# Juleszwanen/oscar_mpc_planner_mr_modification

Hardware: AMD Instinct MI355X
Metric: SQP solves/s (N=20, 8 obs, 8 guesses) at 1/2/4/8 MI355X; max |x−x_ref| (higher is better)
Workload: dtype f64

## Files before the change

### oscar_mpc_planner_mr_modification_amd/csrc/mpcg_sqp.h

```cpp
#pragma once
#include <hip/hip_runtime.h>

#include <type_traits>

#include "mpcg.h"
#include "mpcg_bicycle.h"
#include "mpcg_device.h"

namespace mpcg {

enum { AC_SUCCESS = 0, AC_NAN = 1, AC_MAXITER = 2, AC_MINSTEP = 3, AC_QP_FAILURE = 4 };

__host__ __device__ constexpr int imax(int a, int b) { return a > b ? a : b; }
__host__ __device__ constexpr int sym(int i, int j) { return i >= j ? i * (i + 1) / 2 + j : j * (j + 1) / 2 + i; }
__host__ __device__ constexpr int cpk(int n, int a, int c) { return c * n - c * (c - 1) / 2 + (a - c); }

__host__ __device__ constexpr int lds_b64_cycles(int s, int off, int parts) {
    int total = 0;
    for (int half = 0; half < 2; ++half) {
        int dw[64] = {};
        int n = 0;
        for (int l = 32 * half; l < 32 * half + 32; ++l) {
            const int a = 2 * (s * (l / parts) + off * (l % parts));
            for (int h = 0; h < 2; ++h) {
// ... 40 lines not shown
#endif
    static constexpr int NPTP = (MPCG_P_PAD && MODEL_ != 1 && (64 / (N_ + 1)) >= 3) ? NPT + (NPT & 1) : NPT;
    static constexpr int NB = (HAS_SLACK && NS > 0) ? 4 : 3;
    static constexpr int NBT = NB * (NB + 1) / 2;
    static constexpr int NDH = NZ + NBT + 1;
#ifndef MPCG_PARTS_BIKE
#define MPCG_PARTS_BIKE 2
#endif
    static constexpr int PARTS_MAX = (64 / (N + 1)) >= 3 ? 3 : 2;
    static constexpr int PARTS = MODEL_ == 1 ? (MPCG_PARTS_BIKE < PARTS_MAX ? MPCG_PARTS_BIKE : PARTS_MAX) : PARTS_MAX;
    static_assert((N + 1) * PARTS <= 64, "horizon too long for one wavefront");
    static_assert(NTRI <= 64, "stage block larger than a wavefront");
#if defined(MPCG_NO_QUEUE)
    static constexpr bool QUEUE = false;
#elif defined(MPCG_QUEUE_ALL)
    static constexpr bool QUEUE = true;
#else
    static constexpr bool QUEUE = MODEL_ == 0 && PARTS_MAX == 3;
#endif
    static constexpr int BVS = (NZ + PARTS - 1) / PARTS;
    static constexpr int HS = (NH + PARTS - 1) / PARTS;
    static constexpr int SLOTS = 2 * BVS + HS;
#ifndef MPCG_STORE_IT_MAX
#define MPCG_STORE_IT_MAX 13
#endif
#ifndef MPCG_STORE_IT_MAX2
#ifdef MPCG_STORE_IT_ANY
#define MPCG_STORE_IT_MAX2 12
#else
#define MPCG_STORE_IT_MAX2 0
#endif
#endif
    static constexpr bool STORE_IT = SLOTS <= (PARTS == 3 ? MPCG_STORE_IT_MAX : MPCG_STORE_IT_MAX2);
#ifndef MPCG_BOUNDS_SEL
#define MPCG_BOUNDS_SEL 0
#endif
    static constexpr bool BOUNDS_SEL = MPCG_BOUNDS_SEL > 0;
    static constexpr int NBOX = 2 * NU + 2 * NX;
#ifdef MPCG_LIN_PARAMS_ALL
    static constexpr bool LIN_PARAMS = true;
#else
    static constexpr bool LIN_PARAMS = NS > 0 || N >= 30;
#endif
    static constexpr int DGC = LIN_PARAMS ? 2 : 3;
    static constexpr int NHS = LIN_PARAMS ? (NE > 0 ? NE : 1) : NH;
    static constexpr bool RELOAD_PARAMS = NS > 0 || N >= 30;
    static constexpr int M_TOTAL = 2 * NU + (N - 1) * (NBOX + NH);
    __host__ __device__ static constexpr int blk(int v) {
        return (v >= IX && v <= IPSI) ? v - IX : ((NB == 4 && v == ZSL) ? 3 : -1);
    }
    __host__ __device__ static constexpr int bvar(int b) { return b < 3 ? IX + b : ZSL; }
    static constexpr bool COMPACT = MODEL_ == 1;
#ifndef MPCG_FCONST_N
#define MPCG_FCONST_N 30
#endif
    static constexpr bool FCONST = MODEL_ == 0 && N_ >= MPCG_FCONST_N;
    static constexpr int NFR = COMPACT ? 4 : (FCONST ? 2 : NX), NFC = COMPACT ? NZ - 1 : NZ;
    static constexpr int NHP = COMPACT ? (NZ - 1) * NZ / 2 + 1 : NTRI;
#ifndef MPCG_C3_SPLIT
#define MPCG_C3_SPLIT 0
#endif
#ifndef MPCG_C3_FACFLAT
#define MPCG_C3_FACFLAT 0
#endif
    static constexpr bool CHAIN_SPLIT = !COMPACT || MPCG_C3_SPLIT;
#if defined(MPCG_NO_PAIR)
    static constexpr bool PAIR_WANTED = false;
#elif defined(MPCG_PAIR_ALL)
    static constexpr bool PAIR_WANTED = true;
#else
    static constexpr bool PAIR_WANTED = FCONST && NE_ <= 8;
#endif
    static constexpr bool PAIR_CHAINS = PAIR_WANTED && CHAIN_SPLIT && (N_ + 1) / 2 * NX_ * NX_ <= (N_ + 1) * NDH &&
                                        (N_ + 1) / 2 * NX_ <= 128;
    static constexpr bool FAC_FLAT = !COMPACT || MPCG_C3_FACFLAT;
#ifndef MPCG_REC_P2
#define MPCG_REC_P2 0
#endif
#ifdef MPCG_REC_SELECT
    static constexpr bool REC_FLAT = CHAIN_SPLIT && PARTS == 3;
#else
    static constexpr bool REC_FLAT = CHAIN_SPLIT && (PARTS == 3 || MPCG_REC_P2);
#endif
    static constexpr int QPM_ROWS = 2 * SLOTS * 64;
    static constexpr int QPM = QPM_ROWS + (N + 1) * NZ + N * NX;
    __host__ __device__ static constexpr double slack_coef(int hh) { return (NB == 4 && hh >= NL + NE) ? -1.0 : 0.0; }
};

template <class C, bool LEAN = C::COMPACT, bool GFH = false, int PAD = 0>
struct Lds {
    static constexpr int N = C::N, NX = C::NX, NZ = C::NZ;
    static constexpr int DGS =
        PAD ? lds_stride(C::NHS * C::DGC, C::DGC, C::PARTS, C::DGC % 2 == 0 ? 2 : 1, 3) : C::NHS * C::DGC;
    static constexpr int HDS = PAD ? lds_stride(C::NHS, 1, C::PARTS, 1, 3) : C::NHS;
    static constexpr int PS = PAD == 0   ? C::NPTP
                              : PAD == 2 ? lds_stride(C::NPT + (C::NPT & 1), 0, C::PARTS, 2, 4)
                                         : lds_stride(C::NPTP, 0, C::PARTS, C::NPTP == C::NPT ? 1 : 2, 4);
    double z[N + 1][NZ];
    double H[GFH ? 1 : N + 1][C::NHP];
    double g[N + 1][NZ];
    double F[GFH ? 1 : N][C::NFR][C::NFC];
    double Fst[GFH && !C::COMPACT ? C::NFR : 1][C::NFC];
    double Hst[GFH && !C::COMPACT ? C::NHP : 1];
    double b[N][NX];
    double dH[N + 1][C::NDH];
    double q[N + 1][NZ];
    double dz[N + 1][NZ];
    double ddz[N + 1][NZ];
    double pi_nlp[N][NX];
    double piq[N][NX];
    double pin[LEAN ? 1 : N][NX];
    double rdyn[LEAN ? 1 : N][NX];
    alignas(16) double P[N + 1][PS];
    double Lc[N][C::NLC];
    double Y[N][C::NU][NX];
    double bx[N + 1][NZ];
    double Dg[N][DGS];
    double hd[N][HDS];
    double disc[C::LIN_PARAMS ? N : 1][4];
    double Msc[128];
    double xinit[NX];
    int flag;
};

#ifdef MPCG_LDS_SOLVES_PER_CU
constexpr size_t LDS_QUARTER = 160 * 1024 / MPCG_LDS_SOLVES_PER_CU;
constexpr bool LDS_SMALLEST = true;
#else
constexpr size_t LDS_QUARTER = 160 * 1024 / 4;
constexpr bool LDS_SMALLEST = false;
#endif
template <class C>
__host__ __device__ constexpr bool lds_lean() {
    if (LDS_SMALLEST) return C::COMPACT || sizeof(Lds<C, false>) > LDS_QUARTER;
    return C::COMPACT || (sizeof(Lds<C, false>) > LDS_QUARTER && sizeof(Lds<C, true>) <= LDS_QUARTER);
}
template <class C>
__host__ __device__ constexpr bool lds_gfh() {
#ifdef MPCG_NO_GFH
    return false;
#else
    if (LDS_SMALLEST) return sizeof(Lds<C, lds_lean<C>(), false>) > LDS_QUARTER;
    return sizeof(Lds<C, lds_lean<C>(), false>) > LDS_QUARTER && sizeof(Lds<C, lds_lean<C>(), true>) <= LDS_QUARTER;
#endif
}
template <class C>
__host__ __device__ constexpr int lds_pad() {
#if defined(MPCG_NO_STRIDE_PAD)
    return 0;
#else
#if defined(MPCG_NO_P_ALIGN)
    constexpr bool P_ALIGN = false;
#else
    constexpr bool P_ALIGN = !C::COMPACT;
#endif
    return P_ALIGN && sizeof(Lds<C, lds_lean<C>(), lds_gfh<C>(), 2>) <= LDS_QUARTER ? 2
           : sizeof(Lds<C, lds_lean<C>(), lds_gfh<C>(), 1>) <= LDS_QUARTER         ? 1
                                                                                   : 0;
#endif
}
template <class C>
using LdsOf = Lds<C, lds_lean<C>(), lds_gfh<C>(), lds_pad<C>()>;
template <class C>
__host__ __device__ constexpr size_t gfh_doubles() {
    return lds_gfh<C>() ? (size_t)C::N * C::NFR * C::NFC + (size_t)(C::N + 1) * C::NHP : 0;
}
// ... 333 lines not shown
```

### oscar_mpc_planner_mr_modification_amd/csrc/mpcg_sqp_body.inc

```
    constexpr int N = C::N, PARTS = C::PARTS, NX = C::NX, NZ = C::NZ, NB = C::NB, NBT = C::NBT;
    constexpr int NU = C::NU;
    constexpr int ZS = C::ZSL;
    constexpr int X0 = C::IX, X1 = C::IY, X2 = C::IPSI;
    constexpr bool LEAN = lds_lean<C>();
    constexpr bool GFH = lds_gfh<C>();
#ifndef MPCG_FUSE_BAR
#define MPCG_FUSE_BAR 1
#endif
    constexpr bool FUSE_BAR = MPCG_FUSE_BAR > 0;
#ifndef MPCG_COND
#define MPCG_COND 1
#endif
#ifndef MPCG_ITREF
#define MPCG_ITREF 1
#endif
#ifndef MPCG_MOVE
#define MPCG_MOVE 1
#endif
#ifndef MPCG_RES_SPLIT
#define MPCG_RES_SPLIT 1
#endif
    constexpr bool RES_SPLIT = MPCG_RES_SPLIT > 0 && FUSE_BAR && !C::COMPACT && PARTS > 1 && 2 * NB <= NZ &&
                               ((PARTS == 3 && NX == 5) || MPCG_RES_SPLIT > 1);
    constexpr int DRS = (NX + PARTS - 1) / PARTS;
    static_assert(!(RES_SPLIT && LEAN), "the split passes read the dynamics multipliers from S.pin");
#if defined(MPCG_CENTRED_FLAG)
    constexpr bool CFLAG = MPCG_CENTRED_FLAG > 0;
#else
    constexpr bool CFLAG = !LEAN && !C::HAS_SLACK;
#endif
#ifndef MPCG_MSPLIT
#define MPCG_MSPLIT 0
#endif
    constexpr bool MSPLIT = MPCG_MSPLIT > 0 && C::MODEL == 0;
#ifndef MPCG_PIN_SPLIT
#define MPCG_PIN_SPLIT 0
#endif
    constexpr bool PIN_SPLIT = MPCG_PIN_SPLIT > 0 && RES_SPLIT && !LEAN && C::CHAIN_SPLIT;
    __shared__ LdsOf<C> S;
#ifdef MPCG_LDS_PAD
    __shared__ char lds_pad[MPCG_LDS_PAD];
    if (threadIdx.x == 1000) lds_pad[blockIdx.x % MPCG_LDS_PAD] = 0;
#endif
    if (sol >= batch) return;
    if (blockDim.x != 64) {
        if (threadIdx.x == 0) io.exit_code[sol] = -1;
        return;
    }
#ifdef MPCG_LDS_POISON
    for (int e = threadIdx.x; e < (int)(sizeof(S) / 8); e += 64) ((double*)&S)[e] = __builtin_nan("");
    wave_sync();
#endif
    int lane_ = threadIdx.x;
    if constexpr (C::QUEUE) __asm__ volatile("" : "+v"(lane_));
    const int lane = lane_;
    const int k = lane / PARTS;
    const int part = lane - k * PARTS;
    const bool stage_lane = (part == 0) && (k <= N);
    const int ks = k <= N ? k : N;
    const int kc = k < N ? k : N - 1;
    const int npar = pr.npar;
    constexpr int LAMS = NX + C::NH;
#ifdef MPCG_DIAG_PARAMS_OF
    const double* pbase = io.params + (size_t)(sol % MPCG_DIAG_PARAMS_OF) * N * npar;
#else
    const double* pbase = io.params + (size_t)sol * N * npar;
#endif
    const double* pk = pbase + (size_t)kc * npar;
    (void)stamps;
    constexpr bool SPLIT = MODE != MODE_FUSED;
    double* const gsol = gws + (size_t)(SPLIT ? sol : (int)blockIdx.x) * ws_doubles<C>();
    double* const gF = GFH ? gsol : nullptr;
    double* const g_ddz0 = gsol + gfh_doubles<C>();
    double* const g_pin0 = g_ddz0 + (N + 1) * NZ;
    double* const g_dz0 = g_pin0 + N * NX;
    double* const gH = GFH ? gF + (size_t)N * C::NFR * C::NFC : nullptr;
    auto Fb = [&](int kq) -> double (*)[C::NFC] {
        if constexpr (GFH) return (double (*)[C::NFC])(gF + (size_t)kq * C::NFR * C::NFC);
        else return S.F[kq];
    };
    auto Hb = [&](int kq) -> double* {
        if constexpr (GFH) return gH + (size_t)kq * C::NHP;
        else return S.H[kq];
    };
    STAMP_DECL
    using CB = Carry<C>;
    double* const gcar = g_ddz0 + itref_doubles<C>();
    const bool from_carry = SPLIT && (MODE == MODE_QP || split_it > 0);
    if (from_carry && gcar[CB::META + 1] != 0.0) return;
    auto carry_cp = [&](size_t off, double* a, int n, bool store) {
        for (int e = lane; e < n; e += 64) {
            if (store) gcar[off + e] = a[e];
            else a[e] = gcar[off + e];
        }
    };
    auto carry_lin = [&](bool store) {
        carry_cp(CB::G, &S.g[0][0], (int)(sizeof(S.g) / 8), store);
        carry_cp(CB::B, &S.b[0][0], (int)(sizeof(S.b) / 8), store);
        carry_cp(CB::DG, &S.Dg[0][0], (int)(sizeof(S.Dg) / 8), store);
        carry_cp(CB::HD, &S.hd[0][0], (int)(sizeof(S.hd) / 8), store);
        carry_cp(CB::DISC, &S.disc[0][0], (int)(sizeof(S.disc) / 8), store);
        if constexpr (!GFH) {
            carry_cp(CB::H, &S.H[0][0], (int)(sizeof(S.H) / 8), store);
            carry_cp(CB::F, &S.F[0][0][0], (int)(sizeof(S.F) / 8), store);
        }
    };

    const double* lam_in = io.lam_in ? io.lam_in + (size_t)sol * N * LAMS : nullptr;
// ... 3 lines not shown
    LR.part = part;
    if constexpr (C::BOUNDS_SEL) {
        LR.prb = &pr;
    } else {
#pragma unroll
        for (int j = 0; j < BVS; ++j) {
            const int v = LR.var(j);
            double lo = 0.0, hi = 0.0;
#pragma unroll
            for (int i = 0; i < NZ; ++i)
                if (v == i) { lo = i < NU ? pr.lbu[i] : pr.lbx[i - NU]; hi = i < NU ? pr.ubu[i] : pr.ubx[i - NU]; }
            LR.lo[j] = lo;
            LR.hi[j] = hi;
        }
    }
    auto rowg = [&](int hh, double& a, double& b, double& c) {
        if constexpr (C::LIN_PARAMS) {
            if (hh < C::NL || hh >= C::NL + C::NE) {
                const double* p = hh < C::NL ? pk + pr.i_lin0 + 3 * hh : pk + pr.i_scen0 + 3 * (hh - C::NL - C::NE);
                a = p[0];
                b = p[1];
                c = hh < C::NL ? 0.0 : p[0] * S.disc[k][2] + p[1] * S.disc[k][3];
                return;
            }
            const int he = hh - C::NL;
            a = S.Dg[k][he * C::DGC + 0];
            b = S.Dg[k][he * C::DGC + 1];
            c = a * S.disc[k][2] + b * S.disc[k][3];
        } else {
            a = S.Dg[k][hh * C::DGC + 0]; b = S.Dg[k][hh * C::DGC + 1]; c = S.Dg[k][hh * C::DGC + 2];
        }
    };
    auto rowgap = [&](int hh) -> double {
        if constexpr (C::LIN_PARAMS) {
            const double x = S.z[k][X0], y = S.z[k][X1];
            if (hh < C::NL) {
                const double* p = pk + pr.i_lin0 + 3 * hh;
                return 0.0 - (p[0] * x + p[1] * y - p[2]);
            }
            if (hh >= C::NL + C::NE) {
                const double* p = pk + pr.i_scen0 + 3 * (hh - C::NL - C::NE);
                const double sl = C::HAS_SLACK ? S.z[k][ZS] : 0.0;
                return 0.0 - (p[0] * (x + S.disc[k][0]) + p[1] * (y + S.disc[k][1]) - (p[2] + sl));
            }
            return S.hd[k][hh - C::NL];
        } else {
            return S.hd[k][hh];
        }
    };
    double srow_a = 0.0, srow_v = 0.0;
    if constexpr (C::FCONST) erk_srow(pr, srow_a, srow_v);
    auto FatB = [&](const double (*Fk)[C::NFC], int m, int j) -> double {
        if constexpr (C::FCONST) {
            if (m == 2) return j == 1 ? pr.dt : (j == 4 ? 1.0 : 0.0);
            if (m == 3) return j == 0 ? pr.dt : (j == 5 ? 1.0 : 0.0);
            if (m == 4) return j == 0 ? srow_a : (j == 5 ? srow_v : (j == 6 ? 1.0 : 0.0));
            if (m >= 5) return j == NU + m ? 1.0 : 0.0;
            return Fk[m][j];
        } else if constexpr (C::COMPACT) {
            if (m == 3) return j == bike::ZV ? 1.0 : (j == bike::ZA ? pr.dt : 0.0);
            if (m == 4) return j == bike::ZDELTA ? 1.0 : (j == bike::ZW ? pr.dt : 0.0);
            if (j == ZS) return 0.0;
            return Fk[m < 3 ? m : 3][j < ZS ? j : j - 1];
        } else {
            return Fk[m][j];
        }
    };
    auto HatB = [&](const double* Hk, int i, int j) -> double {
        if constexpr (C::COMPACT) {
            if (i == ZS || j == ZS) return (i == j) ? Hk[C::NHP - 1] : 0.0;
            return Hk[sym(i < ZS ? i : i - 1, j < ZS ? j : j - 1)];
        } else {
            return Hk[sym(i, j)];
        }
    };
    auto Fat = [&](int kq, int m, int j) -> double { return FatB(Fb(kq), m, j); };
    auto Hat = [&](int kq, int i, int j) -> double { return HatB(Hb(kq), i, j); };
    auto rdyn_at = [&](int kq, int i) -> double {
        double a = S.b[kq][i] - S.dz[kq + 1][NU + i];
#pragma unroll
        for (int j = 0; j < NZ; ++j) a += Fat(kq, i, j) * S.dz[kq][j];
        return a;
    };
    Rows<C> R;
#pragma unroll
    for (int r = 0; r < HS; ++r)
        R.nlam[r] = from_carry ? gcar[CB::NLAM + 64 * r + lane]
                               : (lam_in && LR.h_on(r)) ? lam_in[(size_t)k * LAMS + NX + LR.hrow(r)] : 0.0;

    if (from_carry) {
        carry_cp(CB::Z, &S.z[0][0], (N + 1) * NZ, false);
        carry_cp(CB::PI, &S.pi_nlp[0][0], N * NX, false);
    } else {
        const double* w = io.warm + (size_t)sol * (N + 1) * NZ;
        for (int e = lane; e < (N + 1) * NZ; e += 64) (&S.z[0][0])[e] = w[e];
        for (int e = lane; e < N * NX; e += 64)
            (&S.pi_nlp[0][0])[e] = lam_in ? lam_in[(size_t)(e / NX) * LAMS + e % NX] : 0.0;
    }
    if (lane < NX) S.xinit[lane] = io.xinit[(size_t)sol * NX + lane];
    for (int e = lane; e <= N; e += 64) S.dH[e][C::NDH - 1] = 0.0;
    const bool qp_warm = FULL && pr.qp_warm_start == 2;
    const bool sqp_mode = FULL && pr.nlp_solver == MPCG_NLP_SQP;
    bool have_qp = false;
    if (FULL && io.qp_in && !isnan(io.qp_in[(size_t)sol * C::QPM])) {
        const double* q = io.qp_in + (size_t)sol * C::QPM;
#pragma unroll
        for (int sl = 0; sl < C::SLOTS; ++sl) {
            R.t[sl] = q[(2 * sl) * 64 + lane];
            R.l[sl] = q[(2 * sl + 1) * 64 + lane];
        }
        for (int e = lane; e < (N + 1) * NZ; e += 64) (&S.dz[0][0])[e] = q[C::QPM_ROWS + e];
        for (int e = lane; e < N * NX; e += 64) (&S.piq[0][0])[e] = q[C::QPM_ROWS + (N + 1) * NZ + e];
        have_qp = true;
    }
    wave_sync();
    if (lane < NU) S.z[N][lane] = 0.0;
    wave_sync();

    constexpr bool PH = PROF == PROF_HPIPM, PRB = PROF == PROF_ROBUST;
    const bool p_move = PH ? true : PRB ? false : pr.qp_init_move != 0;
    const bool p_cond = PH ? true : PRB ? false : pr.qp_cond_pred_corr != 0;
    const int p_itref = PH ? 2 : PRB ? 0 : pr.qp_itref_corr_max;
    const bool p_sclip = PH ? false : PRB ? true : pr.qp_sigma_clip != 0;
    const bool p_maxit_first = PH ? true : PRB ? false : pr.qp_maxit_first != 0;
    const bool p_pzero = PH ? true : PRB ? false : pr.qp_pivot_zero != 0;
    const double mu_max = PH ? __builtin_inf() : pr.qp_mu_max > 0.0 ? pr.qp_mu_max : __builtin_inf(), tmin = pr.qp_t_min;
    const bool itref_on = MPCG_ITREF && p_itref > 0;
    int acados_status = AC_SUCCESS, qp_status = AC_SUCCESS, sqp_iter = 0, qp_total = 0, n_maxit = 0;
    double res_eq = 0.0;
    double nlp_stat = 0.0, nlp_ineq = 0.0, nlp_comp = 0.0;
    bool nlp_nonfinite = false;
    if (from_carry) {
        res_eq = gcar[CB::META + 0];
        acados_status = (int)gcar[CB::META + 2];
        qp_status = (int)gcar[CB::META + 3];
        sqp_iter = (int)gcar[CB::META + 4];
        qp_total = (int)gcar[CB::META + 5];
        n_maxit = (int)gcar[CB::META + 6];
    }
    bool ended = true;

    for (int it = SPLIT ? split_it : 0; sqp_mode || it < pr.sqp_iters; ++it) {
        if constexpr (C::RELOAD_PARAMS) asm volatile("" : "+v"(pk));
        STAMP_BEGIN();
        if constexpr (MODE == MODE_QP) {
            carry_lin(false);
            if (lane < NX) S.dz[0][NU + lane] = S.xinit[lane] - S.z[0][NU + lane];
        } else {
            double zk[NZ];
#pragma unroll
            for (int i = 0; i < NZ; ++i) zk[i] = S.z[ks][i];
            double hb6[6] = {0, 0, 0, 0, 0, 0};
            if (k >= 1 && k < N) h_rows<C>(pr, pk, zk, LR, R.nlam, hb6, (double (*)[C::DGC])S.Dg[k], S.hd[k], S.disc[C::LIN_PARAMS ? k : 0]);
            STAMP_LAP(10);
            {
                double acc[6];
#pragma unroll
                for (int i = 0; i < 6; ++i) acc[i] = hb6[i];
#pragma unroll
                for (int p = 1; p < PARTS; ++p)
#pragma unroll
                    for (int i = 0; i < 6; ++i) acc[i] += lane_down(hb6[i], p);
#pragma unroll
                for (int i = 0; i < 6; ++i) hb6[i] = acc[i];
            }
            double resl = 0.0;
// ... 253 lines not shown
                }
                if (k < N) {
#pragma unroll
                    for (int i = 0; i < NX; ++i) chk += 0.0 * S.b[k][i];
                }
            }
            nlp_stat = wave_max(vst);
            nlp_ineq = wave_max(vin);
            nlp_comp = wave_max(vcp);
            nlp_nonfinite = !(wave_sum(chk) == 0.0);
            wave_sync();
        }
        if (sqp_mode) {
            if (nlp_nonfinite) {
                acados_status = AC_NAN;
                break;
            }
            if (nlp_stat < pr.nlp_tol && res_eq < pr.nlp_tol && nlp_ineq < pr.nlp_tol && nlp_comp < pr.nlp_tol) {
                acados_status = AC_SUCCESS;
                break;
            }
            if (it >= pr.nlp_max_iter) {
                acados_status = AC_MAXITER;
                break;
            }
        }
        const bool warm_now = qp_warm && have_qp && ((sqp_mode && it > 0) || pr.qp_warm_first);
        bool hcold = false;
        if (warm_now) {
            const double thr = pr.qp_ws_thr;
#pragma unroll
            for (int sl = 0; sl < C::SLOTS; ++sl) {
                if (R.t[sl] < thr) R.t[sl] = thr;
                if (R.l[sl] < thr) R.l[sl] = thr;
                R.pr[sl] = 0.0;
            }
        } else {
        if (stage_lane) {
#pragma unroll
            for (int i = 0; i < NZ; ++i)
                if (!(k == 0 && i >= NU)) S.dz[k][i] = 0.0;
            if (k < N) {
#pragma unroll
                for (int i = 0; i < NX; ++i) S.piq[k][i] = 0.0;
            }
        }
        {
            const double thr0 = pr.qp_thr0, mu0 = pr.qp_mu0;
            const bool mv = MPCG_MOVE && p_move;
            auto cold = [&](int s, double gap) {
                const double t0 = gap > thr0 ? gap : thr0;
                R.t[s] = t0;
                R.l[s] = mu0 / t0;
                R.pr[s] = 0.0;
            };
            wave_sync();
#pragma unroll
            for (int j = 0; j < BVS; ++j) {
                const bool on = LR.box_on(j);
                const double zv = S.z[ks][on ? LR.var(j) : 0];
                const double gl = on ? zv - LR.lo_at(j) : 1.0, gu = on ? LR.hi_at(j) - zv : 1.0;
                if (mv && on) {
                    const bool bl = gl < thr0, bu = gu < thr0;
                    const double ux = bl ? (bu ? 0.5 * (-gl + gu) : -gl + thr0) : (bu ? gu - thr0 : 0.0);
                    S.dz[k][LR.var(j)] = ux;
                }
                cold(2 * j, (mv && gl < thr0) ? thr0 : gl);
                cold(2 * j + 1, (mv && gu < thr0) ? thr0 : gu);
            }
            hcold = mv;
#pragma unroll
            for (int r = 0; r < HS; ++r) {
                const bool on = LR.h_on(r);
                cold(HB + r, on ? rowgap(on ? LR.hrow(r) : 0) : 1.0);
            }
        }
        }
        have_qp = true;
        wave_sync();
        STAMP_END(1);
        int qstat = AC_MAXITER, qit = 0;
        double pinr[LEAN ? NX : 1];
        double Hdz[RES_SPLIT ? BVS : NZ];
        for (;; ++qit) {
            if constexpr (C::RELOAD_PARAMS) asm volatile("" : "+v"(pk));
            STAMP_BEGIN();
            double rs = 0.0, re = 0.0, ri = 0.0, comp = 0.0, cmx = 0.0;
            {
                double zk[NZ], dzk[NZ];
#pragma unroll
                for (int i = 0; i < NZ; ++i) { dzk[i] = S.dz[ks][i]; zk[i] = S.z[ks][i]; }
                double rh[NB], qh[NB], dbh[NBT], rbj[BVS], qbj[BVS];
#pragma unroll
                for (int i = 0; i < NB; ++i) rh[i] = qh[i] = 0.0;
#pragma unroll
                for (int i = 0; i < NBT; ++i) dbh[i] = 0.0;
                auto bar0 = [&](int s, double& coef, double& wgt) {
                    const double l = R.l[s], t = R.t[s], itt = R.it(s);
                    const double rc = l * t;
                    coef = l + (l * R.rin[s] - rc) * itt;
                    wgt = l * itt;
                };
                auto row_res = [&](int s, double ddot, double gap) {
                    const double l = R.l[s], t = R.t[s];
                    const double rin = ddot + t - gap;
                    R.rin[s] = rin;
                    R.set_it(s, frcp(t));
                    ri = fmax(ri, fabs(rin));
                    comp += l * t;
                    cmx = fmax(cmx, l * t);
                };
#pragma unroll
                for (int j = 0; j < BVS; ++j) {
                    double& rb = rbj[j];
                    double& qb = qbj[j];
                    double dd = 0.0;
                    rb = qb = 0.0;
                    if (LR.box_on(j)) {
                        const int v = LR.var(j);
                        const double zv = S.z[k][v], dzv = S.dz[k][v];
                        rb = R.l[2 * j + 1] - R.l[2 * j];
                        row_res(2 * j, -dzv, zv - LR.lo_at(j));
                        row_res(2 * j + 1, dzv, LR.hi_at(j) - zv);
                        if constexpr (FUSE_BAR) {
                            double c0, w0, c1, w1;
                            bar0(2 * j, c0, w0);
                            bar0(2 * j + 1, c1, w1);
                            qb = c1 - c0;
                            dd = w0 + w1;
                        }
                    } else {
                        R.rin[2 * j] = R.rin[2 * j + 1] = 0.0;
                        R.set_it(2 * j, 1.0);
                        R.set_it(2 * j + 1, 1.0);
                    }
                    if (k <= N && LR.var(j) < NZ) {
                        if constexpr (!RES_SPLIT) S.bx[k][LR.var(j)] = rb;
                        if constexpr (FUSE_BAR) {
                            if constexpr (!RES_SPLIT) S.q[k][LR.var(j)] = qb;
                            S.dH[k][LR.var(j)] = dd;
                        }
                    }
                }
#pragma unroll
                for (int r = 0; r < HS; ++r) {
                    if (!LR.h_on(r)) {
                        R.rin[HB + r] = 0.0;
                        R.set_it(HB + r, 1.0);
                        continue;
                    }
                    const int hh = LR.hrow(r);
                    double a, bq, c;
                    rowg(hh, a, bq, c);
                    double dd = a * dzk[X0] + bq * dzk[X1] + c * dzk[X2];
                    if constexpr (NB == 4) dd += C::slack_coef(hh) * dzk[ZS];
                    const double gap = rowgap(hh);
                    if (hcold) {
                        const double t0 = -dd + gap, tt = t0 > pr.qp_thr0 ? t0 : pr.qp_thr0;
                        R.t[HB + r] = tt;
                        R.l[HB + r] = pr.qp_mu0 / tt;
                    }
                    const double l = R.l[HB + r];
                    rh[0] += a * l; rh[1] += bq * l; rh[2] += c * l;
                    if constexpr (NB == 4) rh[3] += C::slack_coef(hh) * l;
                    row_res(HB + r, dd, gap);
                    if constexpr (FUSE_BAR) {
                        double coef, wgt;
                        bar0(HB + r, coef, wgt);
                        double dg[NB];
                        dg[0] = a; dg[1] = bq; dg[2] = c;
                        if constexpr (NB == 4) dg[3] = C::slack_coef(hh);
#pragma unroll
                        for (int i = 0; i < NB; ++i) qh[i] += dg[i] * coef;
#pragma unroll
                        for (int cc = 0; cc < NB; ++cc)
#pragma unroll
                            for (int aa = cc; aa < NB; ++aa) dbh[cpk(NB, aa, cc)] += dg[aa] * wgt * dg[cc];
                    }
                }
                double acc[NB], aq[NB], ab[NBT];
#pragma unroll
                for (int i = 0; i < NB; ++i) { acc[i] = rh[i]; aq[i] = qh[i]; }
#pragma unroll
                for (int i = 0; i < NBT; ++i) ab[i] = dbh[i];
#pragma unroll
                for (int p = 1; p < PARTS; ++p) {
#pragma unroll
                    for (int i = 0; i < NB; ++i) acc[i] += lane_down(rh[i], p);
                    if constexpr (FUSE_BAR) {
#pragma unroll
                        for (int i = 0; i < NB; ++i) aq[i] += lane_down(qh[i], p);
#pragma unroll
                        for (int i = 0; i < NBT; ++i) ab[i] += lane_down(dbh[i], p);
                    }
                }
                if constexpr (RES_SPLIT) {
                    if (stage_lane) {
#pragma unroll
                        for (int i = 0; i < NB; ++i) { S.bx[k][i] = acc[i]; S.bx[k][NB + i] = aq[i]; }
#pragma unroll
                        for (int i = 0; i < NBT; ++i) S.dH[k][NZ + i] = ab[i];
                    }
                    wave_sync();
                    if (k <= N) {
                        double pq[NX];
#pragma unroll
                        for (int m = 0; m < NX; ++m) pq[m] = k < N ? S.piq[k][m] : 0.0;
#pragma unroll
                        for (int j = 0; j < BVS; ++j) {
                            const int v = LR.var(j);
                            if (v >= NZ) continue;
                            double a = 0.0;
#pragma unroll
                            for (int jj = 0; jj < NZ; ++jj) a += Hat(k, v, jj) * dzk[jj];
                            Hdz[j] = a;
                            const int bi = C::blk(v);
                            double rbox = rbj[j];
                            if (bi >= 0) rbox += S.bx[k][bi];
                            double rr = a + S.g[k][v] + rbox;
                            {
                                double qv = a + S.g[k][v] + qbj[j];
                                if (bi >= 0) qv += S.bx[k][NB + bi];
                                S.q[k][v] = qv;
                            }
                            if (k < N) {
#pragma unroll
                                for (int m = 0; m < NX; ++m) rr += Fat(k, m, v) * pq[m];
                            }
                            if (k > 0 && v >= NU) rr -= S.piq[k - 1][v - NU];
                            const bool free_var = (k == N) ? (v >= NU) : ((k == 0) ? (v < NU) : true);
                            if (free_var) rs = fmax(rs, fabs(rr));
                        }
                        if (k < N) {
#pragma unroll
                            for (int jd = 0; jd < DRS; ++jd) {
                                const int i = part + PARTS * jd;
                                if (i >= NX) continue;
                                double a = S.b[k][i] - S.dz[k + 1][NU + i];
#pragma unroll
                                for (int jj = 0; jj < NZ; ++jj) a += Fat(k, i, jj) * dzk[jj];
                                if constexpr (!LEAN) S.rdyn[k][i] = a;
                                re = fmax(re, fabs(a));
                            }
                        }
                    }
                } else {
                wave_sync();
                if (stage_lane) {
                    double rbox[NZ];
#pragma unroll
                    for (int i = 0; i < NZ; ++i) rbox[i] = S.bx[k][i];
#pragma unroll
                    for (int i = 0; i < NB; ++i) rbox[C::bvar(i)] += acc[i];
                    double r[NZ];
#pragma unroll
                    for (int i = 0; i < NZ; ++i) {
                        double a = 0.0;
#pragma unroll
                        for (int j = 0; j < NZ; ++j) a += Hat(k, i, j) * dzk[j];
                        if constexpr (!RES_SPLIT) Hdz[i] = a;
                        r[i] = a + S.g[k][i] + rbox[i];
                    }
                    if constexpr (FUSE_BAR) {
#pragma unroll
                        for (int i = 0; i < NZ; ++i) S.q[k][i] = Hdz[RES_SPLIT ? 0 : i] + S.g[k][i] + S.q[k][i];
#pragma unroll
                        for (int i = 0; i < NB; ++i) S.q[k][C::bvar(i)] += aq[i];
#pragma unroll
                        for (int i = 0; i < NBT; ++i) S.dH[k][NZ + i] = ab[i];
                    }
                    if (k < N) {
#pragma unroll
                        for (int m = 0; m < NX; ++m) {
                            const double pm = S.piq[k][m];
#pragma unroll
                            for (int i = 0; i < NZ; ++i) r[i] += Fat(k, m, i) * pm;
                        }
#pragma unroll
                        for (int i = 0; i < NX; ++i) {
                            double a = S.b[k][i] - S.dz[k + 1][NU + i];
#pragma unroll
                            for (int j = 0; j < NZ; ++j) a += Fat(k, i, j) * dzk[j];
                            if constexpr (!LEAN) S.rdyn[k][i] = a;
                            re = fmax(re, fabs(a));
                        }
                    }
                    if (k > 0) {
#pragma unroll
                        for (int i = 0; i < NX; ++i) r[NU + i] -= S.piq[k - 1][i];
                    }
#pragma unroll
                    for (int i = 0; i < NZ; ++i) {
                        const bool free_var = (k == N) ? (i >= NU) : ((k == 0) ? (i < NU) : true);
                        if (free_var) rs = fmax(rs, fabs(r[i]));
                    }
                }
                }
            }
#ifdef MPCG_TRACE
            rs = wave_max(rs);
            re = wave_max(re);
            ri = wave_max(ri);
#else
            if (itref_on) {
                rs = wave_max(rs);
                re = wave_max(re);
                ri = wave_max(ri);
            } else {
                rs = wave_max(fmax(fmax(rs, re), ri));
                re = ri = rs;
            }
#endif
            if (itref_on) cmx = wave_max(cmx);
            comp = wave_sum(comp);
            hcold = false;
            const double mu = comp / C::M_TOTAL;
#ifdef MPCG_TRACE
            if ((MPCG_TRACE < 0 || sol == MPCG_TRACE) && lane == 0)
                printf("[%d]  ipm it %d rs %.3e re %.3e ri %.3e mu %.3e\n", sol, qit, rs, re, ri, mu);
#endif
            if (!(rs < 1e30) || !(re < 1e30) || !(ri < 1e30) || !(mu < mu_max)) { qstat = AC_NAN; break; }
            if (p_maxit_first && qit >= pr.qp_iter_max) { qstat = AC_MAXITER; break; }
            if (rs < pr.qp_tol && re < pr.qp_tol && ri < pr.qp_tol && mu < pr.qp_tol) { qstat = AC_SUCCESS; break; }
            if (qit >= pr.qp_iter_max) { qstat = AC_MAXITER; break; }
            wave_sync();
            STAMP_END(2);

            double alpha = 1.0, sigma_mu = 0.0, mu_affp = 0.0;
            bool centred = false, redo = false;
            bool refining = false;
            int nref = 0;
            for (int phase = 0; phase < 2; ++phase) {
                STAMP_BEGIN();
                if ((!FUSE_BAR || phase == 1) && !refining) {
                    double qh[NB], dbh[NBT];
#pragma unroll
                    for (int i = 0; i < NB; ++i) qh[i] = 0.0;
#pragma unroll
                    for (int i = 0; i < NBT; ++i) dbh[i] = 0.0;
                    auto bar = [&](int s, double& coef, double& wgt) {
                        const double l = R.l[s], t = R.t[s], itt = R.it(s);
                        const double rc = (phase == 0) ? l * t : l * t + (CFLAG && centred ? 0.0 : R.pr[s]) - sigma_mu;
                        coef = l + (l * R.rin[s] - rc) * itt;
                        wgt = l * itt;
                    };
                    double qbj[BVS];
#pragma unroll
                    for (int j = 0; j < BVS; ++j) {
                        double qb = 0.0, dd = 0.0;
                        if (LR.box_on(j)) {
                            double c0, w0, c1, w1;
                            bar(2 * j, c0, w0);
                            bar(2 * j + 1, c1, w1);
                            qb = c1 - c0;
                            dd = w0 + w1;
                        }
                        qbj[j] = qb;
                        if (k <= N && LR.var(j) < NZ) {
                            if constexpr (!RES_SPLIT) S.bx[k][LR.var(j)] = qb;
                            if (phase == 0) S.dH[k][LR.var(j)] = dd;
                        }
                    }
#pragma unroll
                    for (int r = 0; r < HS; ++r) {
                        if (!LR.h_on(r)) continue;
                        const int hh = LR.hrow(r);
                        double coef, wgt;
                        bar(HB + r, coef, wgt);
                        double dg[NB];
                        rowg(hh, dg[0], dg[1], dg[2]);
                        if constexpr (NB == 4) dg[3] = C::slack_coef(hh);
#pragma unroll
                        for (int i = 0; i < NB; ++i) qh[i] += dg[i] * coef;
                        if (phase == 0) {
#pragma unroll
                            for (int c = 0; c < NB; ++c)
#pragma unroll
                                for (int a = c; a < NB; ++a) dbh[cpk(NB, a, c)] += dg[a] * wgt * dg[c];
                        }
                    }
                    double aq[NB], ab[NBT];
#pragma unroll
                    for (int i = 0; i < NB; ++i) aq[i] = qh[i];
#pragma unroll
                    for (int i = 0; i < NBT; ++i) ab[i] = dbh[i];
#pragma unroll
                    for (int p = 1; p < PARTS; ++p) {
#pragma unroll
                        for (int i = 0; i < NB; ++i) aq[i] += lane_down(qh[i], p);
                        if (phase == 0) {
#pragma unroll
                            for (int i = 0; i < NBT; ++i) ab[i] += lane_down(dbh[i], p);
                        }
                    }
                    if constexpr (RES_SPLIT) {
                        if (stage_lane) {
#pragma unroll
                            for (int i = 0; i < NB; ++i) S.bx[k][i] = aq[i];
// ... 940 lines not shown
                    STAMP_LAP(20);
                    if (phase == 0) {
                        const double aa = fmin(amax, 1.0);
                        double ca = 0.0;
#pragma unroll
                        for (int s = 0; s < C::SLOTS; ++s) {
                            if (!active(s)) continue;
                            double dt, dl;
                            row_step(s, dt, dl);
                            ca += (R.l[s] + aa * dl) * (R.t[s] + aa * dt);
                            R.pr[s] = dt * dl;
                        }
                        ca = wave_sum(ca);
                        const double mu_aff = ca / C::M_TOTAL;
                        mu_affp = mu_aff;
                        double sig = mu_aff / mu;
                        if (p_sclip && sig > 1.0) sig = 1.0;
                        sig = sig * sig * sig;
                        sigma_mu = sig * mu;
                    } else {
                        if (MPCG_COND && p_cond && !centred && nref == 0) {
                            const double ac = fmin(amax, 1.0);
                            cb = wave_sum(cb);
                            cq = wave_sum(cq);
                            const double cc = comp + ac * (cb + ac * cq);
                            if (cc / C::M_TOTAL > 2.0 * mu_affp) {
                                if constexpr (!CFLAG) {
#pragma unroll
                                    for (int s = 0; s < C::SLOTS; ++s) R.pr[s] = 0.0;
                                }
                                centred = redo = true;
                            }
                        }
                        STAMP_LAP(21);
                        bool refine_now = false;
                        if (itref_on && !redo && nref < p_itref) {
                            const double tol = pr.qp_tol;
                            const double thg = fmax(tol, 1e-3 * rs), thb = fmax(tol, 1e-3 * re),
                                         thm = fmax(tol, 1e-3 * cmx);
                            bool fail = false;
                            double rbq[BVS], rh2[NB];
#pragma unroll
                            for (int i = 0; i < NB; ++i) rh2[i] = 0.0;
                            auto row_chk = [&](int sl) -> double {
                                double dt, dl;
                                row_step(sl, dt, dl);
                                const double l = R.l[sl], t = R.t[sl];
                                const double lm = (l * t + (CFLAG && centred ? 0.0 : R.pr[sl]) - smu) + l * dt + t * dl;
                                fail = fail || !(fabs(lm) < thm);
                                return l + dl;
                            };
#pragma unroll
                            for (int j = 0; j < BVS; ++j) {
                                rbq[j] = 0.0;
                                if (LR.box_on(j)) {
                                    const double l0 = row_chk(2 * j);
                                    rbq[j] = row_chk(2 * j + 1) - l0;
                                }
                            }
#pragma unroll
                            for (int r = 0; r < HS; ++r) {
                                if (!LR.h_on(r)) continue;
                                const int hh = LR.hrow(r);
                                const double ln = row_chk(HB + r);
                                double dg[NB];
                                rowg(hh, dg[0], dg[1], dg[2]);
                                if constexpr (NB == 4) dg[3] = C::slack_coef(hh);
#pragma unroll
                                for (int i = 0; i < NB; ++i) rh2[i] += dg[i] * ln;
                            }
                            double ra[NB];
#pragma unroll
                            for (int i = 0; i < NB; ++i) ra[i] = rh2[i];
#pragma unroll
                            for (int p = 1; p < PARTS; ++p)
#pragma unroll
                                for (int i = 0; i < NB; ++i) ra[i] += lane_down(rh2[i], p);
                            if constexpr (RES_SPLIT) {
                                if (stage_lane) {
#pragma unroll
                                    for (int i = 0; i < NB; ++i) S.bx[k][i] = ra[i];
                                }
                                wave_sync();
                                if (k <= N) {
                                    double zt[NZ];
#pragma unroll
                                    for (int i = 0; i < NZ; ++i) zt[i] = S.dz[k][i] + S.ddz[k][i];
#pragma unroll
                                    for (int j = 0; j < BVS; ++j) {
                                        const int v = LR.var(j);
                                        if (v >= NZ) continue;
                                        double a = 0.0;
#pragma unroll
                                        for (int jj = 0; jj < NZ; ++jj) a += Hat(k, v, jj) * zt[jj];
                                        double r = a + S.g[k][v] + rbq[j];
                                        const int bi = C::blk(v);
                                        if (bi >= 0) r += S.bx[k][bi];
                                        if (k < N) {
#pragma unroll
                                            for (int m = 0; m < NX; ++m) r += Fat(k, m, v) * S.pin[k][m];
                                        }
                                        if (k > 0 && v >= NU) r -= S.pin[k - 1][v - NU];
                                        const bool free_var = (k == N) ? (v >= NU) : ((k == 0) ? (v < NU) : true);
                                        if (free_var) fail = fail || !(fabs(r) < thg);
                                    }
                                    if (k < N) {
#pragma unroll
                                        for (int jd = 0; jd < DRS; ++jd) {
                                            const int i = part + PARTS * jd;
                                            if (i >= NX) continue;
                                            double a = S.b[k][i] - (S.dz[k + 1][NU + i] + S.ddz[k + 1][NU + i]);
#pragma unroll
                                            for (int jj = 0; jj < NZ; ++jj) a += Fat(k, i, jj) * zt[jj];
                                            fail = fail || !(fabs(a) < thb);
                                        }
                                    }
                                }
                            } else {
                                if (k <= N) {
#pragma unroll
                                    for (int j = 0; j < BVS; ++j) {
                                        const int v = LR.var(j);
                                        if (v < NZ) S.bx[k][v] = rbq[j];
                                    }
                                }
                                double* const pint = LEAN ? &S.dH[0][0] : &S.pin[0][0];
                                if constexpr (LEAN) {
                                    if (stage_lane && k < N) {
#pragma unroll
                                        for (int i = 0; i < NX; ++i) pint[k * NX + i] = pinr[i];
                                    }
                                }
                                wave_sync();
                                if (stage_lane) {
                                    double zt[NZ];
#pragma unroll
                                    for (int i = 0; i < NZ; ++i) zt[i] = S.dz[k][i] + S.ddz[k][i];
#pragma unroll
                                    for (int i = 0; i < NZ; ++i) {
                                        double a = 0.0;
#pragma unroll
                                        for (int j = 0; j < NZ; ++j) a += Hat(k, i, j) * zt[j];
                                        double r = a + S.g[k][i] + S.bx[k][i];
                                        const int bi = C::blk(i);
                                        if (bi >= 0) r += ra[bi];
                                        if (k < N) {
#pragma unroll
                                            for (int m = 0; m < NX; ++m) r += Fat(k, m, i) * pint[k * NX + m];
                                        }
                                        if (k > 0 && i >= NU) r -= pint[(k - 1) * NX + i - NU];
                                        const bool free_var = (k == N) ? (i >= NU) : ((k == 0) ? (i < NU) : true);
                                        if (free_var) fail = fail || !(fabs(r) < thg);
                                    }
                                    if (k < N) {
#pragma unroll
                                        for (int i = 0; i < NX; ++i) {
                                            double a = S.b[k][i] - (S.dz[k + 1][NU + i] + S.ddz[k + 1][NU + i]);
#pragma unroll
                                            for (int j = 0; j < NZ; ++j) a += Fat(k, i, j) * zt[j];
                                            fail = fail || !(fabs(a) < thb);
                                        }
                                    }
                                }
                                wave_sync();
                                if constexpr (LEAN) {
                                    for (int e = lane; e <= N; e += 64) S.dH[e][C::NDH - 1] = 0.0;
                                }
                            }
                            refine_now = __any(fail);
                            wave_sync();
                        }
                        STAMP_LAP(22);
                        if (refine_now) {
                            auto row_lin = [&](int sl, double& lnew, double& cf) {
                                double dt, dl;
                                row_step(sl, dt, dl);
                                const double l = R.l[sl], t = R.t[sl];
                                const double lm = (l * t + (CFLAG && centred ? 0.0 : R.pr[sl]) - smu) + l * dt + t * dl;
                                cf = -lm * R.it(sl);
                                lnew = l + dl;
                            };
                            double rbq[BVS], cbq[BVS], rh2[NB], ch2[NB];
#pragma unroll
                            for (int i = 0; i < NB; ++i) rh2[i] = ch2[i] = 0.0;
#pragma unroll
                            for (int j = 0; j < BVS; ++j) {
                                rbq[j] = cbq[j] = 0.0;
                                if (LR.box_on(j)) {
                                    double l0, c0, l1, c1;
                                    row_lin(2 * j, l0, c0);
                                    row_lin(2 * j + 1, l1, c1);
                                    rbq[j] = l1 - l0;
                                    cbq[j] = c1 - c0;
                                }
                            }
#pragma unroll
                            for (int r = 0; r < HS; ++r) {
                                if (!LR.h_on(r)) continue;
                                const int hh = LR.hrow(r);
                                double ln, cf, dg[NB];
                                row_lin(HB + r, ln, cf);
                                rowg(hh, dg[0], dg[1], dg[2]);
                                if constexpr (NB == 4) dg[3] = C::slack_coef(hh);
#pragma unroll
                                for (int i = 0; i < NB; ++i) { rh2[i] += dg[i] * ln; ch2[i] += dg[i] * cf; }
                            }
                            double ra[NB], ca[NB];
#pragma unroll
                            for (int i = 0; i < NB; ++i) { ra[i] = rh2[i]; ca[i] = ch2[i]; }
#pragma unroll
                            for (int p = 1; p < PARTS; ++p)
#pragma unroll
                                for (int i = 0; i < NB; ++i) { ra[i] += lane_down(rh2[i], p); ca[i] += lane_down(ch2[i], p); }
                            if (k <= N) {
#pragma unroll
                                for (int j = 0; j < BVS; ++j) {
                                    const int v = LR.var(j);
                                    if (v < NZ) { S.bx[k][v] = rbq[j]; S.q[k][v] = cbq[j]; }
                                }
                            }
                            double* const pint = LEAN ? &S.dH[0][0] : &S.pin[0][0];
                            if constexpr (LEAN) {
                                if (stage_lane && k < N) {
#pragma unroll
                                    for (int i = 0; i < NX; ++i) pint[k * NX + i] = pinr[i];
                                }
                            }
                            wave_sync();
                            if (stage_lane) {
                                double zt[NZ];
#pragma unroll
                                for (int i = 0; i < NZ; ++i) zt[i] = S.dz[k][i] + S.ddz[k][i];
#pragma unroll
                                for (int i = 0; i < NZ; ++i) {
                                    double a = 0.0;
#pragma unroll
                                    for (int j = 0; j < NZ; ++j) a += Hat(k, i, j) * zt[j];
                                    double r = a + S.g[k][i] + S.bx[k][i];
                                    const int bi = C::blk(i);
                                    if (bi >= 0) r += ra[bi];
                                    if (k < N) {
#pragma unroll
                                        for (int m = 0; m < NX; ++m) r += Fat(k, m, i) * pint[k * NX + m];
                                    }
                                    if (k > 0 && i >= NU) r -= pint[(k - 1) * NX + i - NU];
                                    const bool free_var = (k == N) ? (i >= NU) : ((k == 0) ? (i < NU) : true);
                                    double q2 = r + S.q[k][i];
                                    if (bi >= 0) q2 += ca[bi];
                                    S.q[k][i] = free_var ? q2 : 0.0;
                                }
                                if constexpr (!LEAN) {
                                    if (k < N) {
#pragma unroll
                                        for (int i = 0; i < NX; ++i) {
                                            double a = S.b[k][i] - (S.dz[k + 1][NU + i] + S.ddz[k + 1][NU + i]);
#pragma unroll
                                            for (int j = 0; j < NZ; ++j) a += Fat(k, i, j) * zt[j];
                                            S.rdyn[k][i] = a;
                                        }
                                    }
                                }
                            }
                            {
                                ++nref;
                                for (int e = lane; e < (N + 1) * NZ; e += 64) g_ddz0[e] = (&S.ddz[0][0])[e];
                                if constexpr (LEAN) {
                                    if (stage_lane && k < N) {
#pragma unroll
                                        for (int i = 0; i < NX; ++i) g_pin0[k * NX + i] = pinr[i];
                                    }
                                    wave_sync();
                                    for (int e = lane; e < (N + 1) * NZ; e += 64) {
                                        const double d = (&S.dz[0][0])[e];
                                        g_dz0[e] = d;
                                        (&S.dz[0][0])[e] = d + (&S.ddz[0][0])[e];
                                    }
                                } else {
                                    for (int e = lane; e < N * NX; e += 64) g_pin0[e] = (&S.pin[0][0])[e];
                                }
                                redo = refining = true;
#ifdef MPCG_TRACE
                                if ((MPCG_TRACE < 0 || sol == MPCG_TRACE) && lane == 0) printf("[%d]  itref %d\n", sol, nref);
#endif
                            }
                            wave_sync();
                            if constexpr (LEAN) {
                                for (int e = lane; e <= N; e += 64) S.dH[e][C::NDH - 1] = 0.0;
                            }
                        }
                        STAMP_LAP(23);
                        alpha = 0.995 * amax;
                        if (alpha > 1.0) alpha = 1.0;
                        if (!redo && alpha >= 1e-12) {
#pragma unroll
                            for (int s = 0; s < C::SLOTS; ++s) {
                                if (!active(s)) continue;
                                double dt, dl;
                                row_step(s, dt, dl);
                                const double tn = R.t[s] + alpha * dt, ln = R.l[s] + alpha * dl;
                                R.t[s] = tn < tmin ? tmin : tn;
                                R.l[s] = ln < tmin ? tmin : ln;
                            }
                        }
                    }
                }
                wave_sync();
                STAMP_END(7);
                if (redo) {
                    redo = false;
                    phase = 0;
                }
            }
            if (qstat == AC_NAN) break;
            if (alpha < 1e-12) { qstat = AC_MINSTEP; ++qit; break; }
            STAMP_BEGIN();
            if (RES_SPLIT && !LEAN) {
                if (k <= N) {
#pragma unroll
                    for (int j = 0; j < BVS; ++j) {
                        const int v = LR.var(j);
                        if (v < NZ) S.dz[k][v] += alpha * S.ddz[k][v];
                    }
                    if (k < N) {
#pragma unroll
                        for (int jd = 0; jd < DRS; ++jd) {
                            const int i = part + PARTS * jd;
                            if (i < NX) S.piq[k][i] += alpha * (S.pin[k][i] - S.piq[k][i]);
                        }
                    }
                }
            } else if (stage_lane) {
#pragma unroll
                for (int i = 0; i < NZ; ++i) S.dz[k][i] += alpha * S.ddz[k][i];
                if (k < N) {
#pragma unroll
                    for (int i = 0; i < NX; ++i) {
                        if constexpr (LEAN) S.piq[k][i] += alpha * (pinr[i] - S.piq[k][i]);
                        else S.piq[k][i] += alpha * (S.pin[k][i] - S.piq[k][i]);
                    }
                }
            }
            wave_sync();
            STAMP_END(8);
        }
        wave_sync();
        qp_status = qstat;
        qp_total += qit;
        ++sqp_iter;
        n_maxit += qstat == AC_MAXITER;
        if (qstat != AC_SUCCESS && qstat != AC_MAXITER) {
            acados_status = AC_QP_FAILURE;
            break;
        }
        if (stage_lane) {
#pragma unroll
            for (int i = 0; i < NZ; ++i) S.z[k][i] += S.dz[k][i];
            if (k == N) {
#pragma unroll
                for (int u = 0; u < NU; ++u) S.z[N][u] = 0.0;
            }
            if (k < N) {
#pragma unroll
                for (int i = 0; i < NX; ++i) S.pi_nlp[k][i] = S.piq[k][i];
            }
        }
#pragma unroll
        for (int r = 0; r < HS; ++r)
            if (LR.h_on(r)) R.nlam[r] = R.l[HB + r];
        wave_sync();
        acados_status = AC_SUCCESS;
        if (!sqp_mode && qstat != AC_SUCCESS) break;
        if constexpr (MODE == MODE_QP) {
            ended = it + 1 >= pr.sqp_iters;
            break;
        }
    }
    if constexpr (MODE == MODE_QP) {
        if (lane == 0) {
            gcar[CB::META + 1] = ended ? 1.0 : 0.0;
            gcar[CB::META + 2] = acados_status;
            gcar[CB::META + 3] = qp_status;
            gcar[CB::META + 4] = sqp_iter;
            gcar[CB::META + 5] = qp_total;
            gcar[CB::META + 6] = n_maxit;
        }
        if (!ended) {
            carry_cp(CB::Z, &S.z[0][0], (N + 1) * NZ, true);
            carry_cp(CB::PI, &S.pi_nlp[0][0], N * NX, true);
#pragma unroll
            for (int r = 0; r < HS; ++r) gcar[CB::NLAM + 64 * r + lane] = R.nlam[r];
            return;
        }
    }

    double Lk = 0.0;
    if (stage_lane && k < N) {
        double zz[NZ], gd[NZ], Hd[NZ][NZ];
#pragma unroll
        for (int i = 0; i < NZ; ++i) zz[i] = S.z[k][i];
        if constexpr (C::MODEL == 1) Lk = bike::stage_cost(pr, pk, k, zz, gd, Hd, false);
        else Lk = stage_cost<NX>(pr, pk, zz, gd, Hd, false);
    }
    const double pobj = wave_sum(Lk);
    double* xo = io.xtraj + (size_t)sol * (N + 1) * NX;
    for (int e = lane; e < (N + 1) * NX; e += 64) xo[e] = S.z[e / NX][NU + e % NX];
    double* uo = io.utraj + (size_t)sol * N * NU;
    for (int e = lane; e < N * NU; e += 64) uo[e] = S.z[e / NU][e % NU];
    if (io.lam_out) {
        double* lo = io.lam_out + (size_t)sol * N * LAMS;
        for (int e = lane; e < N * NX; e += 64) lo[(size_t)(e / NX) * LAMS + e % NX] = S.pi_nlp[e / NX][e % NX];
// ... 41 lines not shown
```

Baseline: 548,200.

## Carry predicted next-iterate residuals from iterative-refinement check into next QP iteration

During the iterative-refinement residual check, the code now also evaluates the Hessian-times-step, stationarity and dynamics residuals at the predicted next iterate (step fraction 0.995*amax capped at 1). It stores them in S.q, S.rdyn and Hdz. When refinement is not triggered, the next QP iteration reuses these carried values instead of recomputing the stationarity and dynamics residuals. The goal is to remove a redundant residual pass per interior-point iteration. The cost is extra FMAs in the check and a reliance on the actual alpha matching the predicted step; any mismatch would make the carried residuals inconsistent.

```diff
diff --git a/oscar_mpc_planner_mr_modification_amd/csrc/mpcg_sqp.h b/oscar_mpc_planner_mr_modification_amd/csrc/mpcg_sqp.h
--- a/oscar_mpc_planner_mr_modification_amd/csrc/mpcg_sqp.h
+++ b/oscar_mpc_planner_mr_modification_amd/csrc/mpcg_sqp.h
@@ -146,6 +146,10 @@
 #else
     static constexpr bool REC_FLAT = CHAIN_SPLIT && (PARTS == 3 || MPCG_REC_P2);
 #endif
+#ifndef MPCG_RES_CARRY
+#define MPCG_RES_CARRY 1
+#endif
+    static constexpr bool RES_CARRY = MPCG_RES_CARRY > 0 && MODEL_ == 0 && PARTS == 3 && NX_ == 5;
     static constexpr int QPM_ROWS = 2 * SLOTS * 64;
     static constexpr int QPM = QPM_ROWS + (N + 1) * NZ + N * NX;
     __host__ __device__ static constexpr double slack_coef(int hh) { return (NB == 4 && hh >= NL + NE) ? -1.0 : 0.0; }
diff --git a/oscar_mpc_planner_mr_modification_amd/csrc/mpcg_sqp_body.inc b/oscar_mpc_planner_mr_modification_amd/csrc/mpcg_sqp_body.inc
--- a/oscar_mpc_planner_mr_modification_amd/csrc/mpcg_sqp_body.inc
+++ b/oscar_mpc_planner_mr_modification_amd/csrc/mpcg_sqp_body.inc
@@ -24,6 +24,7 @@
                                ((PARTS == 3 && NX == 5) || MPCG_RES_SPLIT > 1);
     constexpr int DRS = (NX + PARTS - 1) / PARTS;
     static_assert(!(RES_SPLIT && LEAN), "the split passes read the dynamics multipliers from S.pin");
+    constexpr bool RES_CARRY = C::RES_CARRY && RES_SPLIT && !LEAN && MPCG_ITREF > 0;
 #if defined(MPCG_CENTRED_FLAG)
     constexpr bool CFLAG = MPCG_CENTRED_FLAG > 0;
 #else
@@ -193,6 +194,7 @@
         for (int j = 0; j < NZ; ++j) a += Fat(kq, i, j) * S.dz[kq][j];
         return a;
     };
+    auto stepped = [](double x, double a, double dx) -> double { return x + a * dx; };
     Rows<C> R;
 #pragma unroll
     for (int r = 0; r < HS; ++r)
@@ -612,6 +614,7 @@
         int qstat = AC_MAXITER, qit = 0;
         double pinr[LEAN ? NX : 1];
         double Hdz[RES_SPLIT ? BVS : NZ];
+        bool carried = false;
         for (;; ++qit) {
             if constexpr (C::RELOAD_PARAMS) asm volatile("" : "+v"(pk));
             STAMP_BEGIN();
@@ -732,7 +735,31 @@
                         for (int i = 0; i < NBT; ++i) S.dH[k][NZ + i] = ab[i];
                     }
                     wave_sync();
-                    if (k <= N) {
+                    if (RES_CARRY && carried) {
+                        if (k <= N) {
+#pragma unroll
+                            for (int j = 0; j < BVS; ++j) {
+                                const int v = LR.var(j);
+                                if (v >= NZ) continue;
+                                const int bi = C::blk(v);
+                                double rbox = rbj[j];
+                                if (bi >= 0) rbox += S.bx[k][bi];
+                                double qv = Hdz[j] + S.g[k][v] + qbj[j];
+                                if (bi >= 0) qv += S.bx[k][NB + bi];
+                                const double rr = S.q[k][v] + rbox;
+                                const bool free_var = (k == N) ? (v >= NU) : ((k == 0) ? (v < NU) : true);
+                                S.q[k][v] = qv;
+                                if (free_var) rs = fmax(rs, fabs(rr));
+                            }
+                            if (k < N) {
+#pragma unroll
+                                for (int jd = 0; jd < DRS; ++jd) {
+                                    const int i = part + PARTS * jd;
+                                    if (i < NX) re = fmax(re, fabs(S.rdyn[k][i]));
+                                }
+                            }
+                        }
+                    } else if (k <= N) {
                         double pq[NX];
 #pragma unroll
                         for (int m = 0; m < NX; ++m) pq[m] = k < N ? S.piq[k][m] : 0.0;
@@ -844,6 +871,7 @@
             if (itref_on) cmx = wave_max(cmx);
             comp = wave_sum(comp);
             hcold = false;
+            carried = false;
             const double mu = comp / C::M_TOTAL;
 #ifdef MPCG_TRACE
             if ((MPCG_TRACE < 0 || sol == MPCG_TRACE) && lane == 0)
@@ -1950,25 +1978,60 @@
                                     for (int i = 0; i < NB; ++i) S.bx[k][i] = ra[i];
                                 }
                                 wave_sync();
+                                double an = 0.995 * amax;
+                                if (an > 1.0) an = 1.0;
                                 if (k <= N) {
-                                    double zt[NZ];
-#pragma unroll
-                                    for (int i = 0; i < NZ; ++i) zt[i] = S.dz[k][i] + S.ddz[k][i];
+                                    double zt[NZ], zn[RES_CARRY ? NZ : 1], pn[RES_CARRY ? NX : 1];
+#pragma unroll
+                                    for (int i = 0; i < NZ; ++i) {
+                                        const double d = S.dz[k][i], dd = S.ddz[k][i];
+                                        zt[i] = d + dd;
+                                        if constexpr (RES_CARRY) zn[i] = stepped(d, an, dd);
+                                    }
+                                    if constexpr (RES_CARRY) {
+                                        if (k < N) {
+#pragma unroll
+                                            for (int m = 0; m < NX; ++m) {
+                                                const double p = S.piq[k][m];
+                                                pn[m] = stepped(p, an, S.pin[k][m] - p);
+                                            }
+                                        }
+                                    }
 #pragma unroll
                                     for (int j = 0; j < BVS; ++j) {
                                         const int v = LR.var(j);
                                         if (v >= NZ) continue;
-                                        double a = 0.0;
-#pragma unroll
-                                        for (int jj = 0; jj < NZ; ++jj) a += Hat(k, v, jj) * zt[jj];
-                                        double r = a + S.g[k][v] + rbq[j];
+                                        double a = 0.0, a2 = 0.0;
+#pragma unroll
+                                        for (int jj = 0; jj < NZ; ++jj) {
+                                            const double h = Hat(k, v, jj);
+                                            a += h * zt[jj];
+                                            if constexpr (RES_CARRY) a2 += h * zn[jj];
+                                        }
+                                        const double gv = S.g[k][v];
+                                        double r = a + gv + rbq[j];
+                                        double c = a2 + gv;
                                         const int bi = C::blk(v);
                                         if (bi >= 0) r += S.bx[k][bi];
                                         if (k < N) {
 #pragma unroll
-                                            for (int m = 0; m < NX; ++m) r += Fat(k, m, v) * S.pin[k][m];
+                                            for (int m = 0; m < NX; ++m) {
+                                                const double f = Fat(k, m, v);
+                                                r += f * S.pin[k][m];
+                                                if constexpr (RES_CARRY) c += f * pn[m];
+                                            }
                                         }
-                                        if (k > 0 && v >= NU) r -= S.pin[k - 1][v - NU];
+                                        if (k > 0 && v >= NU) {
+                                            r -= S.pin[k - 1][v - NU];
+                                            if constexpr (RES_CARRY) {
+                                                const double p = S.piq[k - 1][v - NU];
+                                                c -= stepped(p, an, S.pin[k - 1][v - NU] - p);
+                                            }
+                                        }
+                                        if constexpr (RES_CARRY) {
+                                            Hdz[j] = a2;
+                                            S.q[k][v] = c;
+                                        }
                                         const bool free_var = (k == N) ? (v >= NU) : ((k == 0) ? (v < NU) : true);
                                         if (free_var) fail = fail || !(fabs(r) < thg);
                                     }
@@ -1977,10 +2040,17 @@
                                         for (int jd = 0; jd < DRS; ++jd) {
                                             const int i = part + PARTS * jd;
                                             if (i >= NX) continue;
-                                            double a = S.b[k][i] - (S.dz[k + 1][NU + i] + S.ddz[k + 1][NU + i]);
-#pragma unroll
-                                            for (int jj = 0; jj < NZ; ++jj) a += Fat(k, i, jj) * zt[jj];
+                                            const double d = S.dz[k + 1][NU + i], dd = S.ddz[k + 1][NU + i];
+                                            double a = S.b[k][i] - (d + dd);
+                                            double a2 = S.b[k][i] - (RES_CARRY ? stepped(d, an, dd) : 0.0);
+#pragma unroll
+                                            for (int jj = 0; jj < NZ; ++jj) {
+                                                const double f = Fat(k, i, jj);
+                                                a += f * zt[jj];
+                                                if constexpr (RES_CARRY) a2 += f * zn[jj];
+                                            }
                                             fail = fail || !(fabs(a) < thb);
+                                            if constexpr (RES_CARRY) S.rdyn[k][i] = a2;
                                         }
                                     }
                                 }
@@ -2036,6 +2106,7 @@
                                 }
                             }
                             refine_now = __any(fail);
+                            if constexpr (RES_CARRY) carried = !refine_now;
                             wave_sync();
                         }
                         STAMP_LAP(22);
@@ -2187,13 +2258,16 @@
 #pragma unroll
                     for (int j = 0; j < BVS; ++j) {
                         const int v = LR.var(j);
-                        if (v < NZ) S.dz[k][v] += alpha * S.ddz[k][v];
+                        if (v < NZ) S.dz[k][v] = stepped(S.dz[k][v], alpha, S.ddz[k][v]);
                     }
                     if (k < N) {
 #pragma unroll
                         for (int jd = 0; jd < DRS; ++jd) {
                             const int i = part + PARTS * jd;
-                            if (i < NX) S.piq[k][i] += alpha * (S.pin[k][i] - S.piq[k][i]);
+                            if (i < NX) {
+                                const double p = S.piq[k][i];
+                                S.piq[k][i] = stepped(p, alpha, S.pin[k][i] - p);
+                            }
                         }
                     }
                 }
```

Result: faster. 556,000, median of 6 (+1.4%).
